# Fuad-HH/PumiUMTally

Measured on AMD Instinct MI355X. Metric: particle-steps/sec, higher is better.
Workload: dtype fp64; 1 GPU; model=track-length-tally-walk, mesh_tets=998250, global_batch=10000000, particles_per_gpu=10000000, parallelism=dp1-replicated-mesh, nscores=1, comm=torch-rccl, ngroups=1, device=gpu, lost_particles=0

## Files before the change

### csrc/core/engine.h

```cpp
#pragma once

#include "mesh.h"
#include "walk.h"

#include <cstdint>
#include <cstdlib>
#include <stdexcept>
#include <memory>
#include <string>
#include <vector>

namespace pumitally {

struct EngineStats {
  int64_t lost_particles = 0;
  int64_t moves = 0;
  int64_t relocated = 0;
  int64_t loose_localizations = 0;
  int64_t origins_elided = 0;
  int64_t origin_bytes_uploaded = 0;
  double origin_pass_seconds = 0.0;
  int64_t collisions_scored = 0;
  int64_t collision_misses = 0;
};

constexpr int kMaxLostRecords = 16;

class Engine {
public:
  virtual ~Engine() = default;

  virtual int64_t num_particles() const = 0;
  virtual const Mesh &mesh() const = 0;

  virtual void copy_initial_position(const double *positions, int64_t n) = 0;

  virtual void move(const double *origin, const double *dest,
                    const int8_t *flying, const double *weights, int64_t n,
                    const uint16_t *groups = nullptr,
                    const double *responses = nullptr) = 0;

  virtual void move_continue(const double *dest, const int8_t *flying,
                             const double *weights, int64_t n,
                             const uint16_t *groups = nullptr,
                             const double *responses = nullptr) {
    move(nullptr, dest, flying, weights, n, groups, responses);
  }

  virtual void move_device(const double *d_origin, const double *d_dest,
                           const int8_t *d_flying, const double *d_weights,
                           int64_t n, const uint16_t *d_groups = nullptr,
                           const double *d_responses = nullptr) {
    (void)d_origin; (void)d_dest; (void)d_flying; (void)d_weights; (void)n;
    (void)d_groups; (void)d_responses;
// ... 105 lines not shown
  virtual void set_particle_state(const double *pos, const int32_t *elem,
                                  const uint8_t *escaped, int64_t n) = 0;

  virtual void synchronize() {}

  struct DeviceMeshView {
    const Plane *planes = nullptr;
    const int32_t *nbr = nullptr;
    GridView grid{};
    void *stream = nullptr;
  };
  virtual bool device_mesh(DeviceMeshView *out) const {
    (void)out;
    return false;
  }

  int max_steps = 0;
  int ngroups = 1;
  int nscores = 1;

  bool reflective = false;

  bool linear = false;

  bool face_currents = false;

  bool collision_tallies = false;

  bool walk_fp32 = false;

  bool origin_elide = true;
  int origin_threads = 8;
  int64_t origin_chunk = 0;

protected:
  [[noreturn]] static void throw_not_linear() {
    throw std::runtime_error(
        "linear moment tallies are off: create the engine with linear=true");
  }
  [[noreturn]] static void throw_not_currents() {
    throw std::runtime_error(
        "face-current tallies are off: create the engine with currents=true");
  }
  [[noreturn]] static void throw_not_collisions() {
    throw std::runtime_error(
        "collision tallies are off: create the engine with collisions=true");
  }
};

inline bool default_walk_fp32() {
  const char *s = getenv("PUMITALLY_WALK");
  return s && std::string(s) == "fp32";
}

inline bool default_origin_elide() {
  const char *s = getenv("PUMITALLY_ORIGIN_ELIDE");
  return !s || atoi(s) != 0;
}

inline int default_origin_threads() {
  const char *s = getenv("PUMITALLY_ORIGIN_THREADS");
  const int k = s ? atoi(s) : 8;
  return k < 1 ? 1 : (k > 16 ? 16 : k);
}

inline int64_t default_origin_chunk() {
  const char *s = getenv("PUMITALLY_ORIGIN_CHUNK");
  const int64_t c = s ? (int64_t)atoll(s) : 0;
  return c < 0 ? 0 : c;
}

inline bool default_reflective() {
  const char *s = getenv("PUMITALLY_BC");
  return s && std::string(s) == "reflective";
}

inline double loc_tol_rel() {
  const char *s = getenv("PUMITALLY_LOC_TOL");
  return s ? atof(s) : 1e-10;
}

std::unique_ptr<Engine> make_cpu_engine(Mesh mesh, int64_t num_particles,
                                        int ngroups = 1, int nscores = 1,
                                        bool linear = false,
                                        bool currents = false,
                                        bool collisions = false);

std::unique_ptr<Engine> make_gpu_engine(Mesh mesh, int64_t num_particles,
                                        int device, int ngroups = 1,
                                        int nscores = 1, bool linear = false,
                                        bool currents = false,
                                        bool collisions = false);

inline void check_tally_options(bool linear, bool currents) {
  if (linear && currents)
    throw std::invalid_argument(
        "currents=true cannot be combined with linear=true (not implemented)");
}

std::vector<double> normalize_flux(const Mesh &m, const std::vector<double> &flux);
// ... 8 lines not shown
```

### csrc/core/origin_delta.cpp

```cpp
#include "origin_delta.h"

#include <algorithm>
#include <atomic>
#include <cstring>

#if defined(__SSE2__) && !defined(__HIP_DEVICE_COMPILE__)
#include <emmintrin.h>
#define PT_HAVE_STREAM_STORE 1
#else
#define PT_HAVE_STREAM_STORE 0
#endif

namespace pumitally {

int origin_delta_clamp_threads(int requested) {
  return std::max(1, std::min(requested, kOriginDeltaMaxThreads));
}

OriginDeltaPool::OriginDeltaPool(int nthreads)
    : nthreads_(origin_delta_clamp_threads(nthreads)) {
  for (int t = 1; t < nthreads_; ++t)
    threads_.emplace_back([this, t] { worker(t); });
}

// ... 73 lines not shown
  _mm_sfence();
#endif
}

template <bool NT>
int64_t delta_part(const double *origin, const double *dest, double *shadow,
                   int64_t lo, int64_t hi, int32_t *pidx, double *pxyz,
                   int64_t cap) {
  int64_t count = 0;
  for (int64_t i = lo; i < hi; ++i) {
    const double *o = origin + i * 3;
    double *s = shadow + i * 3;
    const uint64_t diff = (load_bits(o) ^ load_bits(s)) |
                          (load_bits(o + 1) ^ load_bits(s + 1)) |
                          (load_bits(o + 2) ^ load_bits(s + 2));
    if (diff) {
      if (count < cap) {
        pidx[count] = (int32_t)i;
        pxyz[count * 3] = o[0];
        pxyz[count * 3 + 1] = o[1];
        pxyz[count * 3 + 2] = o[2];
      }
      ++count;
    }
    const double *d = dest + i * 3;
    store_bits<NT>(s, load_bits(d));
    store_bits<NT>(s + 1, load_bits(d + 1));
    store_bits<NT>(s + 2, load_bits(d + 2));
  }
  if (NT) store_fence();
  return count;
}

template <bool NT>
void copy_part(const double *dest, double *shadow, int64_t lo, int64_t hi) {
  for (int64_t k = lo * 3; k < hi * 3; ++k)
    store_bits<NT>(shadow + k, load_bits(dest + k));
  if (NT) store_fence();
}

}

int64_t origin_delta_block(int64_t len, int nthreads) {
  const int64_t t = origin_delta_clamp_threads(nthreads);
  const int64_t b = (len + 4 * t - 1) / (4 * t);
  return std::max<int64_t>(1, std::min(b, kMaxBlock));
}

int64_t origin_delta_patch_capacity(int64_t len, int nthreads) {
  if (len <= 0) return 0;
  const int64_t block = origin_delta_block(len, nthreads);
  const int64_t full = len / block, tail = len % block;
  return full * seg_capacity(block) + (tail ? seg_capacity(tail) : 0);
}

OriginDeltaResult origin_delta_pass(OriginDeltaPool &pool,
                                    const double *origin, const double *dest,
                                    double *shadow, int64_t lo, int64_t hi,
                                    int32_t *patch_idx, double *patch_xyz,
                                    bool nontemporal) {
  OriginDeltaResult r;
  const int64_t len = hi - lo;
  if (len <= 0) return r;
  r.block = origin_delta_block(len, pool.nthreads());
  r.nsegs = (len + r.block - 1) / r.block;
  r.seg_off.resize(r.nsegs);
  r.seg_cap.resize(r.nsegs);
  r.seg_count.assign(r.nsegs, 0);
  for (int64_t b = 0; b < r.nsegs; ++b) {
    const int64_t blen = std::min(r.block, len - b * r.block);
    r.seg_off[b] = b * seg_capacity(r.block);
    r.seg_cap[b] = seg_capacity(blen);
  }
  std::atomic<int64_t> next{0};
  const std::function<void(int)> job = [&](int) {
    for (;;) {
      const int64_t b = next.fetch_add(1, std::memory_order_relaxed);
      if (b >= r.nsegs) return;
      const int64_t a = lo + b * r.block;
      const int64_t e = std::min(hi, a + r.block);
      int32_t *pi = patch_idx + r.seg_off[b];
      double *px = patch_xyz + r.seg_off[b] * 3;
      r.seg_count[b] =
          nontemporal
              ? delta_part<true>(origin, dest, shadow, a, e, pi, px,
                                 r.seg_cap[b])
              : delta_part<false>(origin, dest, shadow, a, e, pi, px,
                                  r.seg_cap[b]);
    }
  };
  pool.run(job);
  for (int64_t b = 0; b < r.nsegs; ++b) {
    r.changed += r.seg_count[b];
    if (r.seg_count[b] > r.seg_cap[b]) r.overflow = true;
  }
  return r;
}

void origin_delta_compact(const OriginDeltaResult &r, int32_t *patch_idx,
                          double *patch_xyz) {
  int64_t out = 0;
  for (int64_t b = 0; b < r.nsegs; ++b) {
    const int64_t cnt = r.seg_count[b];
    if (cnt && r.seg_off[b] != out) {
      std::memmove(patch_idx + out, patch_idx + r.seg_off[b],
                   cnt * sizeof(int32_t));
      std::memmove(patch_xyz + out * 3, patch_xyz + r.seg_off[b] * 3,
                   cnt * 3 * sizeof(double));
    }
    out += cnt;
  }
}

void origin_delta_seed(OriginDeltaPool &pool, const double *dest,
                       double *shadow, int64_t lo, int64_t hi,
                       bool nontemporal) {
  const int64_t len = hi - lo;
  if (len <= 0) return;
  const int64_t block = origin_delta_block(len, pool.nthreads());
  const int64_t nblocks = (len + block - 1) / block;
  std::atomic<int64_t> next{0};
  const std::function<void(int)> job = [&](int) {
    for (;;) {
      const int64_t b = next.fetch_add(1, std::memory_order_relaxed);
      if (b >= nblocks) return;
      const int64_t a = lo + b * block;
      const int64_t e = std::min(hi, a + block);
      if (nontemporal)
        copy_part<true>(dest, shadow, a, e);
      else
        copy_part<false>(dest, shadow, a, e);
    }
  };
  pool.run(job);
}

}
```

### csrc/core/origin_delta.h

```cpp
#pragma once

#include <condition_variable>
#include <cstdint>
#include <functional>
#include <mutex>
#include <thread>
#include <vector>

namespace pumitally {

constexpr int kOriginDeltaMaxThreads = 16;

int origin_delta_clamp_threads(int requested);

class OriginDeltaPool {
public:
  explicit OriginDeltaPool(int nthreads);
  ~OriginDeltaPool();
  OriginDeltaPool(const OriginDeltaPool &) = delete;
  OriginDeltaPool &operator=(const OriginDeltaPool &) = delete;

  int nthreads() const { return nthreads_; }
  void run(const std::function<void(int)> &f);

// ... 6 lines not shown
  std::condition_variable cv_start_, cv_done_;
  const std::function<void(int)> *job_ = nullptr;
  uint64_t generation_ = 0;
  int pending_ = 0;
  bool stop_ = false;
};

struct OriginDeltaResult {
  int64_t block = 0;
  int64_t nsegs = 0;
  std::vector<int64_t> seg_off, seg_cap;
  std::vector<int64_t> seg_count;
  int64_t changed = 0;
  bool overflow = false;
};

int64_t origin_delta_block(int64_t len, int nthreads);

int64_t origin_delta_patch_capacity(int64_t len, int nthreads);

OriginDeltaResult origin_delta_pass(OriginDeltaPool &pool,
                                    const double *origin, const double *dest,
                                    double *shadow, int64_t lo, int64_t hi,
                                    int32_t *patch_idx, double *patch_xyz,
                                    bool nontemporal = false);

void origin_delta_compact(const OriginDeltaResult &r, int32_t *patch_idx,
                          double *patch_xyz);

void origin_delta_seed(OriginDeltaPool &pool, const double *dest,
                       double *shadow, int64_t lo, int64_t hi,
                       bool nontemporal = false);

}
```

### csrc/hip/engine_gpu.hip

```cpp
#include "../core/engine.h"
#include "../core/origin_delta.h"
#include "../core/tally_sink.h"
#include "../core/walk.h"
#include "hip_util.h"

#include <hip/hip_runtime.h>
#include <hipcub/hipcub.hpp>

#include <algorithm>
#include <type_traits>
#include <array>
#include <chrono>
#include <cstdio>
#include <cstdlib>
#include <cstring>
#include <memory>
#include <stdexcept>
#include <string>
#include <vector>

namespace pumitally {

namespace {

// ... 691 lines not shown
      d_flying_[p].allocate(n_);
      d_weights_[p].allocate(n_);
      if (ngroups > 1) d_groups_[p].allocate(n_);
    }

    sort_every_ = sort_every();
    if (sort_every_ > 0) {
      d_keys_.allocate(n_);
      d_keys2_.allocate(n_);
      d_vals_.allocate(n_);
      d_order_.allocate(n_);
      d_pos2_.allocate(n_ * 3);
      d_elem2_.allocate(n_);
      d_esc2_.allocate(n_);
      d_s2c2_.allocate(n_);
      size_t bytes = 0;
      PT_HIP_CHECK(hipcub::DeviceRadixSort::SortPairs(
          nullptr, bytes, d_keys_.get(), d_keys2_.get(), d_vals_.get(),
          d_order_.get(), (int)n_, 0, 64, s_comp_));
      sorttmp_bytes_ = bytes;
      d_sorttmp_.allocate(bytes ? bytes : 1);
      const Vec3 ext = mesh_.bbox_hi - mesh_.bbox_lo;
      sort_scale_ = Vec3{ext.x > 0 ? 2097151.0 / ext.x : 0.0,
                         ext.y > 0 ? 2097151.0 / ext.y : 0.0,
                         ext.z > 0 ? 2097151.0 / ext.z : 0.0};
    }

    loc_tol_ = loc_tol_rel() * norm(mesh_.bbox_hi - mesh_.bbox_lo);
    walk_fp32 = default_walk_fp32();
    reflective = default_reflective();
    origin_elide = default_origin_elide();
    origin_threads = default_origin_threads();
    origin_chunk = default_origin_chunk();
    const Vec3 c0 = mesh_.nelems > 0 ? mesh_.centroid(0) : Vec3{0, 0, 0};
    k_init_particles<<<grid_blocks(n_), kBlock, 0, s_comp_>>>(
        d_pos_, d_elem_, d_escaped_, d_s2c_, n_, c0.x, c0.y, c0.z);
    PT_HIP_CHECK(hipGetLastError());
    PT_HIP_CHECK(hipStreamSynchronize(s_comp_));
  }

  ~GpuEngine() override {
    (void)hipSetDevice(device_);
    (void)hipDeviceSynchronize();
  }

  int64_t num_particles() const override { return n_; }
  const Mesh &mesh() const override { return mesh_; }

  void copy_initial_position(const double *p, int64_t n) override {
    check_n(n);
    PT_HIP_CHECK(hipSetDevice(device_));
    sync();
    stage(p, n * 3 * sizeof(double), d_origin_[0], s_copy_);
    PT_HIP_CHECK(hipStreamSynchronize(s_copy_));
    k_iota<<<grid_blocks(n_), kBlock, 0, s_comp_>>>(d_s2c_, n_);
    k_locate<<<grid_blocks(n_), kBlock, 0, s_comp_>>>(
        d_planes_, grid_view_, d_origin_[0], d_pos_, d_elem_, d_escaped_,
        d_loose_, n_, loc_tol_);
    PT_HIP_CHECK(hipGetLastError());
    if (sort_every_ > 0) spatial_sort();
    moves_since_sort_ = 0;
    PT_HIP_CHECK(hipStreamSynchronize(s_comp_));
  }

  void move(const double *origin, const double *dest, const int8_t *flying,
            const double *weights, int64_t n,
            const uint16_t *groups = nullptr,
            const double *responses = nullptr) override {
    check_n(n);
    PT_HIP_CHECK(hipSetDevice(device_));
    const int steps = max_steps > 0 ? max_steps : default_max_steps(mesh_);
    const int p = (int)(parity_++ & 1);
    PT_HIP_CHECK(hipStreamWaitEvent(s_copy_, kernels_done_[p], 0));
    if (responses && !d_resp_[p]) d_resp_[p].allocate(n_ * nscores);
    const bool probe = origin && origin_elide && n > 0 && elide_skip_ == 0;
    if (probe && shadow_valid_) {
      stage_elided(p, origin, dest, flying, weights, groups, responses, n);
    } else {
      if (origin) {
        stage(origin, n * 3 * sizeof(double), d_origin_[p], s_copy_);
        stats_.origin_bytes_uploaded += n * 3 * (int64_t)sizeof(double);
      }
      stage_inputs(p, dest, flying, weights, groups, responses, n);
      shadow_valid_ = false;
      if (probe) {
        ensure_elide_host(n);
        const auto t0 = std::chrono::steady_clock::now();
        origin_delta_seed(*delta_pool_, dest, shadow_.get(), 0, n,
                          false);
        stats_.origin_pass_seconds += seconds_since(t0);
        shadow_valid_ = true;
      } else if (origin && origin_elide && elide_skip_ > 0) {
        --elide_skip_;
      }
    }
    PT_HIP_CHECK(hipEventRecord(copy_ev_[p], s_copy_));
    PT_HIP_CHECK(hipStreamWaitEvent(s_comp_, copy_ev_[p], 0));
    launch_move_chunks(origin ? d_origin_[p] : nullptr, d_dest_[p],
                       d_flying_[p], d_weights_[p],
                       groups ? d_groups_[p] : nullptr,
                       responses ? d_resp_[p] : nullptr, n, steps);
    PT_HIP_CHECK(hipEventRecord(kernels_done_[p], s_comp_));
    maybe_resort();
    PT_HIP_CHECK(hipStreamSynchronize(s_copy_));
    stats_.moves++;
  }

  void move_device(const double *d_origin, const double *d_dest,
                   const int8_t *d_flying, const double *d_weights, int64_t n,
                   const uint16_t *d_groups = nullptr,
                   const double *d_responses = nullptr) override {
    check_n(n);
    PT_HIP_CHECK(hipSetDevice(device_));
    const int steps = max_steps > 0 ? max_steps : default_max_steps(mesh_);
    launch_move_chunks(d_origin, d_dest, d_flying, d_weights, d_groups,
                       d_responses, n, steps);
    maybe_resort();
    stats_.moves++;
  }

  void score_collisions(const int8_t *active, const double *weights,
                        int64_t n, const uint16_t *groups = nullptr,
                        const double *responses = nullptr) override {
// ... 390 lines not shown
    PT_HIP_CHECK(hipStreamSynchronize(s_comp_));
    PT_HIP_CHECK(hipMemcpy(d_pos_, pos, n * 3 * sizeof(double), hipMemcpyHostToDevice));
    PT_HIP_CHECK(hipMemcpy(d_elem_, elem, n * sizeof(int32_t), hipMemcpyHostToDevice));
    PT_HIP_CHECK(hipMemcpy(d_escaped_, escaped, n, hipMemcpyHostToDevice));
    moves_since_sort_ = sort_every_;
  }

  void synchronize() override { sync(); }

  bool device_mesh(DeviceMeshView *out) const override {
    out->planes = d_planes_;
    out->nbr = d_nbr_;
    out->grid = grid_view_;
    out->stream = (void *)s_comp_;
    return true;
  }

private:
  void check_n(int64_t n) const {
    if (n != n_) throw std::runtime_error("particle count mismatch");
  }

  void sync() const {
    PT_HIP_CHECK(hipStreamSynchronize(s_copy_));
    PT_HIP_CHECK(hipStreamSynchronize(s_comp_));
  }

  void stage(const void *src, size_t bytes, void *dst, hipStream_t s) {
    PT_HIP_CHECK(hipMemcpyAsync(dst, src, bytes, hipMemcpyHostToDevice, s));
  }

  void stage_inputs(int p, const double *dest, const int8_t *flying,
                    const double *weights, const uint16_t *groups,
                    const double *responses, int64_t n) {
    stage(dest, n * 3 * sizeof(double), d_dest_[p], s_copy_);
    stage(flying, n * sizeof(int8_t), d_flying_[p], s_copy_);
    stage(weights, n * sizeof(double), d_weights_[p], s_copy_);
    if (groups && d_groups_[p])
      stage(groups, n * sizeof(uint16_t), d_groups_[p], s_copy_);
    if (responses)
      stage(responses, n * nscores * sizeof(double), d_resp_[p], s_copy_);
  }

  static constexpr int kElideBackoffFirst = 16;
  static constexpr int kElideBackoffMax = 256;

  static double seconds_since(std::chrono::steady_clock::time_point t0) {
    return std::chrono::duration<double>(std::chrono::steady_clock::now() -
                                         t0)
        .count();
  }

  int64_t elide_chunk(int64_t n) const {
    if (origin_chunk > 0) return std::max<int64_t>(origin_chunk, 64);
    return std::max<int64_t>((int64_t)262144, (n + 1) / 2);
  }

  void ensure_elide_host(int64_t n) {
    const int want = origin_delta_clamp_threads(origin_threads);
    if (!delta_pool_ || delta_pool_->nthreads() != want)
      delta_pool_ = std::make_unique<OriginDeltaPool>(want);
    if (!shadow_) shadow_.reset(new double[n * 3]);
  }

  void ensure_patch(int64_t need) {
    if (need <= patch_cap_) return;
    PT_HIP_CHECK(hipStreamSynchronize(s_copy_));
    patch_cap_ = 0;
    h_patch_idx_.reset();
    h_patch_xyz_.reset();
    d_patch_idx_.reset();
    d_patch_xyz_.reset();
    h_patch_idx_.allocate(need);
    h_patch_xyz_.allocate(need * 3);
    d_patch_idx_.allocate(need);
    d_patch_xyz_.allocate(need * 3);
    patch_cap_ = need;
  }

  void stage_elided(int p, const double *origin, const double *dest,
                    const int8_t *flying, const double *weights,
                    const uint16_t *groups, const double *responses,
                    int64_t n) {
    ensure_elide_host(n);
    const int nthreads = delta_pool_->nthreads();
    const int64_t chunk = elide_chunk(n);
    int64_t need = 0;
    for (int64_t lo = 0; lo < n; lo += chunk)
      need += origin_delta_patch_capacity(std::min(chunk, n - lo), nthreads);
    ensure_patch(need);
    shadow_valid_ = false;
    k_copy_doubles<<<grid_blocks(n * 3 / 2), kBlock, 0, s_copy_>>>(
        d_dest_[p ^ 1], d_origin_[p], n * 3);
    PT_HIP_CHECK(hipGetLastError());
    stage_inputs(p, dest, flying, weights, groups, responses, n);
    int64_t region = 0, uploaded = 0;
    for (int64_t lo = 0; lo < n; lo += chunk) {
      const int64_t hi = std::min(n, lo + chunk);
      const int64_t len = hi - lo;
      const int64_t cap = origin_delta_patch_capacity(len, nthreads);
      if (region + cap > patch_cap_)
        throw std::runtime_error("origin elision: patch region overflow");
      int32_t *hidx = h_patch_idx_ + region;
      double *hxyz = h_patch_xyz_ + region * 3;
      const auto t0 = std::chrono::steady_clock::now();
      const OriginDeltaResult r = origin_delta_pass(
          *delta_pool_, origin, dest, shadow_.get(), lo, hi, hidx, hxyz,
          false);
      stats_.origin_pass_seconds += seconds_since(t0);
      if (r.overflow || r.changed * 2 > len) {
        stage(origin + lo * 3, len * 3 * sizeof(double),
              d_origin_[p] + lo * 3, s_copy_);
        uploaded += len;
      } else if (r.changed > 0) {
        origin_delta_compact(r, hidx, hxyz);
        stage(hidx, r.changed * sizeof(int32_t), d_patch_idx_ + region,
              s_copy_);
        stage(hxyz, r.changed * 3 * sizeof(double),
              d_patch_xyz_ + region * 3, s_copy_);
        k_scatter_origins<<<grid_blocks(r.changed), kBlock, 0, s_copy_>>>(
            d_patch_idx_ + region, d_patch_xyz_ + region * 3, d_origin_[p],
            r.changed);
        PT_HIP_CHECK(hipGetLastError());
        uploaded += r.changed;
      }
      region += cap;
    }
    stats_.origins_elided += n - uploaded;
    stats_.origin_bytes_uploaded += uploaded * 3 * (int64_t)sizeof(double);
    shadow_valid_ = true;
    if (uploaded * 2 > n) {
      elide_skip_ = elide_backoff_;
      elide_backoff_ = std::min(elide_backoff_ * 2, kElideBackoffMax);
    } else {
      elide_backoff_ = kElideBackoffFirst;
    }
  }

  void launch_walk_raw(int64_t n, const double *pos, const double *dest,
                       const int32_t *elem, const double *weights,
                       double *out_pos, int32_t *out_elem, int8_t *out_status,
// ... 84 lines not shown
    }
  }

  template <class T>
  std::pair<std::vector<int32_t>, std::vector<T>> fetch(const T *dev,
                                                        int comps) const {
    sync();
    std::vector<int32_t> s2c(n_);
    std::vector<T> v(n_ * comps);
    PT_HIP_CHECK(hipMemcpy(s2c.data(), d_s2c_, n_ * sizeof(int32_t),
                           hipMemcpyDeviceToHost));
    PT_HIP_CHECK(hipMemcpy(v.data(), dev, n_ * comps * sizeof(T),
                           hipMemcpyDeviceToHost));
    return {std::move(s2c), std::move(v)};
  }

  Mesh mesh_;
  int64_t n_;
  int64_t fsz_ = 0;
  int device_ = 0;
  double loc_tol_ = 1e-12;
  int slices_ = 1;
  int sort_every_ = 0;
  int64_t moves_since_sort_ = 0;
  uint64_t parity_ = 0;
  Vec3 sort_scale_{0, 0, 0};

  std::unique_ptr<double[]> shadow_;
  bool shadow_valid_ = false;
  std::unique_ptr<OriginDeltaPool> delta_pool_;
  int64_t patch_cap_ = 0;
  int elide_skip_ = 0;
  int elide_backoff_ = kElideBackoffFirst;

  Stream s_copy_, s_comp_;
  std::array<Event, 2> copy_ev_;
  std::array<Event, 2> kernels_done_;
  Stream s_score_;
  Event score_copied_, score_done_;
  bool score_queued_ = false;

  PinnedBuffer<int32_t> h_patch_idx_;
  PinnedBuffer<double> h_patch_xyz_;
  DeviceBuffer<int32_t> d_patch_idx_;
  DeviceBuffer<double> d_patch_xyz_;

  DeviceBuffer<Plane> d_planes_;
  DeviceBuffer<Plane32> d_planes32_;
  DeviceBuffer<int32_t> d_nbr_, d_cell_start_, d_cell_tets_;
  GridView grid_view_{};

  DeviceBuffer<double> d_pos_;
  DeviceBuffer<int32_t> d_elem_;
  DeviceBuffer<uint8_t> d_escaped_;
  DeviceBuffer<int32_t> d_s2c_;
  DeviceBuffer<double> d_flux_;
  DeviceBuffer<unsigned long long> d_lost_, d_loose_;
  DeviceBuffer<double> d_lostrec_;
  DeviceBuffer<double> d_origin_[2], d_dest_[2], d_weights_[2], d_resp_[2];
  DeviceBuffer<int8_t> d_flying_[2];
  DeviceBuffer<uint16_t> d_groups_[2];
  DeviceBuffer<double> d_bsum_, d_bsq_;
  DeviceBuffer<double> d_inv_h_, d_moments_, d_msum_;
  DeviceBuffer<double> d_cur_, d_csum_, d_csq_;
  bool cur_keyed_ = false;
  DeviceBuffer<double> d_coll_, d_collsum_, d_collsq_;
  DeviceBuffer<unsigned long long> d_coll_counts_;
  bool coll_agg_ = true;
  DeviceBuffer<int8_t> sc_active_;
  DeviceBuffer<double> sc_weights_, sc_resp_;
  DeviceBuffer<uint16_t> sc_groups_;
  ScorePointsScratch sp_;
  DeviceBuffer<uint32_t> d_face_bc_;
  DeviceBuffer<int32_t> d_pidx_, d_pelem_;
// ... 35 lines not shown
```

### csrc/pybind/module.cpp

```cpp
#include <pybind11/numpy.h>
#include <pybind11/pybind11.h>
#include <pybind11/stl.h>

#include "../api/PumiTally.h"
#include "../comm/comm.h"
#include "../core/engine.h"
#include "../core/partition_engine.h"

#include <hip/hip_runtime.h>

#include <cstdint>
#include <cstring>
#include <memory>
#include <thread>
#include <vector>

namespace py = pybind11;
using namespace pumitally;

namespace {

bool have_gpu() {
  int n = 0;
  if (hipGetDeviceCount(&n) != hipSuccess) {
// ... 673 lines not shown
           py::arg("ngroups") = 1, py::arg("nscores") = 1,
           py::arg("linear") = false, py::arg("currents") = false,
           py::arg("collisions") = false)
      .def_property_readonly(
          "collision_tallies",
          [](const PyEngine &e) { return e.eng->collision_tallies; })
      .def_property_readonly("linear",
                             [](const PyEngine &e) { return e.eng->linear; })
      .def_property_readonly(
          "face_currents",
          [](const PyEngine &e) { return e.eng->face_currents; })
      .def_property_readonly(
          "reflective", [](const PyEngine &e) { return e.eng->reflective; })
      .def_property_readonly("ngroups",
                             [](const PyEngine &e) { return e.eng->ngroups; })
      .def_property_readonly("nscores",
                             [](const PyEngine &e) { return e.eng->nscores; })
      .def_property_readonly("num_particles",
                             [](const PyEngine &e) { return e.eng->num_particles(); })
      .def_property_readonly("is_gpu", [](const PyEngine &e) { return e.gpu; })
      .def_property(
          "max_steps", [](const PyEngine &e) { return e.eng->max_steps; },
          [](PyEngine &e, int v) { e.eng->max_steps = v; })
      .def_property(
          "origin_elide", [](const PyEngine &e) { return e.eng->origin_elide; },
          [](PyEngine &e, bool v) { e.eng->origin_elide = v; })
      .def_property(
          "origin_threads",
          [](const PyEngine &e) { return e.eng->origin_threads; },
          [](PyEngine &e, int v) { e.eng->origin_threads = v; })
      .def_property(
          "origin_chunk", [](const PyEngine &e) { return e.eng->origin_chunk; },
          [](PyEngine &e, int64_t v) { e.eng->origin_chunk = v; })
      .def("copy_initial_position",
           [](PyEngine &e, py::array_t<double, py::array::c_style | py::array::forcecast> p) {
             if ((int64_t)p.size() != e.eng->num_particles() * 3)
               throw std::runtime_error("positions must have size 3*num_particles");
             e.eng->copy_initial_position(p.data(), e.eng->num_particles());
           })
      .def("move",
           [](PyEngine &e, py::array_t<double, py::array::c_style> origin,
              py::array_t<double, py::array::c_style> dest,
              py::array_t<int8_t, py::array::c_style> flying,
              py::array_t<double, py::array::c_style> weights,
              py::object groups, py::object responses) {
             const int64_t n = e.eng->num_particles();
             if ((int64_t)origin.size() != n * 3 || (int64_t)dest.size() != n * 3 ||
                 (int64_t)flying.size() != n || (int64_t)weights.size() != n)
               throw std::runtime_error("move: array size mismatch");
             const uint16_t *gp = nullptr;
             py::array_t<uint16_t, py::array::c_style | py::array::forcecast> garr;
             if (!groups.is_none()) {
               garr = groups.cast<py::array_t<uint16_t, py::array::c_style | py::array::forcecast>>();
               if ((int64_t)garr.size() != n)
                 throw std::runtime_error("move: groups size mismatch");
               gp = garr.data();
             }
             const double *rp = nullptr;
             py::array_t<double, py::array::c_style | py::array::forcecast> rarr;
             if (!responses.is_none()) {
               rarr = responses.cast<py::array_t<double, py::array::c_style | py::array::forcecast>>();
               if ((int64_t)rarr.size() != n * e.eng->nscores)
                 throw std::runtime_error("move: responses size must be n*nscores");
               rp = rarr.data();
             }
             py::gil_scoped_release nogil;
// ... 248 lines not shown
           py::arg("groups_ptr") = 0, py::arg("responses_ptr") = 0)
      .def("collisions", [](const PyEngine &e) { return vec_to_np(e.eng->collisions()); })
      .def("collision_sum", [](const PyEngine &e) { return vec_to_np(e.eng->collision_sum()); })
      .def("collision_sum_sq", [](const PyEngine &e) { return vec_to_np(e.eng->collision_sum_sq()); })
      .def("set_collisions",
           [](PyEngine &e, py::array_t<double, py::array::c_style | py::array::forcecast> c) {
             e.eng->set_collisions(c.data(), (int64_t)c.size());
           })
      .def("set_particle_state",
           [](PyEngine &e, py::array_t<double, py::array::c_style | py::array::forcecast> pos,
              py::array_t<int32_t, py::array::c_style | py::array::forcecast> elem,
              py::array_t<uint8_t, py::array::c_style | py::array::forcecast> escaped) {
             const int64_t n = e.eng->num_particles();
             if ((int64_t)pos.size() != n * 3 || (int64_t)elem.size() != n ||
                 (int64_t)escaped.size() != n)
               throw std::runtime_error("set_particle_state: size mismatch");
             e.eng->set_particle_state(pos.data(), elem.data(), escaped.data(), n);
           })
      .def("end_batch", [](PyEngine &e) { py::gil_scoped_release ng; e.eng->end_batch(); })
      .def("batch_sum", [](const PyEngine &e) { return vec_to_np(e.eng->batch_sum()); })
      .def("batch_sum_sq", [](const PyEngine &e) { return vec_to_np(e.eng->batch_sum_sq()); })
      .def_property_readonly("num_batches",
                             [](const PyEngine &e) { return e.eng->num_batches(); })
      .def("stats", [](const PyEngine &e) {
        const EngineStats &s = e.eng->stats();
        py::dict d;
        d["lost_particles"] = s.lost_particles;
        d["moves"] = s.moves;
        d["relocated"] = s.relocated;
        d["loose_localizations"] = s.loose_localizations;
        d["origins_elided"] = s.origins_elided;
        d["origin_bytes_uploaded"] = s.origin_bytes_uploaded;
        d["origin_pass_seconds"] = s.origin_pass_seconds;
        d["collisions_scored"] = s.collisions_scored;
        d["collision_misses"] = s.collision_misses;
        return d;
      })
      .def("lost_records", [](const PyEngine &e) {
        auto v = e.eng->lost_records();
        auto arr = vec_to_np(std::move(v));
        return arr.reshape({(py::ssize_t)(arr.size() / 4), (py::ssize_t)4});
      });

  py::class_<PumiTally>(m, "PumiTally")
      .def(py::init([](const std::string &mesh, int32_t n) {
        int argc = 0;
        char **argv = nullptr;
        return new PumiTally(mesh, n, argc, argv);
      }))
      .def("copy_initial_position",
           [](PumiTally &t, py::array_t<double, py::array::c_style | py::array::forcecast> p) {
             t.CopyInitialPosition((double *)p.data(), (int32_t)p.size());
           })
      .def("move_to_next_location",
           [](PumiTally &t, py::array_t<double, py::array::c_style> origin,
              py::array_t<double, py::array::c_style> dest,
              py::array_t<int8_t, py::array::c_style> flying,
              py::array_t<double, py::array::c_style> weights) {
             t.MoveToNextLocation((double *)origin.data(), (double *)dest.data(),
                                  (int8_t *)flying.mutable_data(),
                                  (double *)weights.data(), (int32_t)origin.size());
           })
      .def("write_tally_results", &PumiTally::WriteTallyResults)
      .def("tally_times", [](const PumiTally &t) {
        py::dict d;
        d["initialization_time"] = t.InitializationTime();
// ... 6 lines not shown
```

### pumiumtally_amd/__init__.py

```python
from __future__ import annotations

import os as _os

if _os.environ.get("PUMITALLY_NO_TORCH", "0") != "1":
    try:
        import torch as _torch
    except ImportError:
        pass


def _load_core():
    try:
        from . import _core
        return _core
    except ImportError as e:
        if _os.environ.get("PUMITALLY_AUTOBUILD", "1") == "1":
            from ._build import build
            build()
            from . import _core
            return _core
        raise ImportError(
            "pumiumtally_amd._core is not built. Run "
            "`python -m pumiumtally_amd._build` first."
        ) from e
# ... 74 lines not shown
        return self._eng.is_gpu

    @property
    def max_steps(self) -> int:
        return self._eng.max_steps

    @max_steps.setter
    def max_steps(self, v: int) -> None:
        self._eng.max_steps = v

    @property
    def origin_elide(self) -> bool:
        return self._eng.origin_elide

    @origin_elide.setter
    def origin_elide(self, v: bool) -> None:
        self._eng.origin_elide = bool(v)

    @property
    def origin_threads(self) -> int:
        return self._eng.origin_threads

    @origin_threads.setter
    def origin_threads(self, v: int) -> None:
        self._eng.origin_threads = int(v)

    @property
    def origin_chunk(self) -> int:
        return self._eng.origin_chunk

    @origin_chunk.setter
    def origin_chunk(self, v: int) -> None:
        self._eng.origin_chunk = int(v)

    def copy_initial_position(self, positions):
        self._eng.copy_initial_position(positions)

    def move(self, origin, dest, flying, weights, groups=None,
             responses=None):
        self._eng.move(origin, dest, flying, weights, groups, responses)

    def move_continue(self, dest, flying, weights, groups=None,
                      responses=None):
        self._eng.move_continue(dest, flying, weights, groups, responses)

    def move_from_device(self, dest, flying, weights, origin=None,
                         sync_torch=True, groups=None, responses=None):
        def ptr(t, dtype, numel):
            return _device_ptr(t, dtype, numel, "move_from_device")

        n = self.num_particles
        if sync_torch:
            _sync_torch()
        self._eng.move_device(
            ptr(origin, "<f8", n * 3), ptr(dest, "<f8", n * 3),
            ptr(flying, "|i1", n), ptr(weights, "<f8", n),
            ptr(groups, "<u2", n), ptr(responses, "<f8", n * self.nscores))

    def walk_raw(self, pos, dest, elem, weights, groups=None,
                 responses=None, in_t=None, in_prev=None, resume=False):
        return self._eng.walk_raw(pos, dest, elem, weights, groups,
                                  responses, in_t, in_prev, resume)

    def synchronize(self):
        self._eng.synchronize()

# ... 396 lines not shown
```

Measured before the change: 1.401 billion particle-steps/s.

## Echo uploaded dest back to pinned host and elide unchanged flying/weight uploads

```diff
diff --git a/csrc/core/engine.h b/csrc/core/engine.h
--- a/csrc/core/engine.h
+++ b/csrc/core/engine.h
@@ -20,6 +20,11 @@
   int64_t origins_elided = 0;
   int64_t origin_bytes_uploaded = 0;
   double origin_pass_seconds = 0.0;
+  double origin_echo_wait_seconds = 0.0;
+  int64_t origin_echo_fallbacks = 0;
+  int64_t weight_bytes_uploaded = 0;
+  int64_t flying_bytes_uploaded = 0;
+  double input_pass_seconds = 0.0;
   int64_t collisions_scored = 0;
   int64_t collision_misses = 0;
 };
@@ -191,6 +196,9 @@
   bool origin_elide = true;
   int origin_threads = 8;
   int64_t origin_chunk = 0;
+  bool origin_echo = true;
+  bool input_elide = true;
+  int64_t input_block = 0;
 
 protected:
   [[noreturn]] static void throw_not_linear() {
@@ -225,6 +233,22 @@
 
 inline int64_t default_origin_chunk() {
   const char *s = getenv("PUMITALLY_ORIGIN_CHUNK");
+  const int64_t c = s ? (int64_t)atoll(s) : 0;
+  return c < 0 ? 0 : c;
+}
+
+inline bool default_origin_echo() {
+  const char *s = getenv("PUMITALLY_ORIGIN_ECHO");
+  return !s || atoi(s) != 0;
+}
+
+inline bool default_input_elide() {
+  const char *s = getenv("PUMITALLY_INPUT_ELIDE");
+  return !s || atoi(s) != 0;
+}
+
+inline int64_t default_input_block() {
+  const char *s = getenv("PUMITALLY_INPUT_BLOCK");
   const int64_t c = s ? (int64_t)atoll(s) : 0;
   return c < 0 ? 0 : c;
 }
diff --git a/csrc/core/origin_delta.cpp b/csrc/core/origin_delta.cpp
--- a/csrc/core/origin_delta.cpp
+++ b/csrc/core/origin_delta.cpp
@@ -129,6 +129,28 @@
   return count;
 }
 
+int64_t compare_part(const double *origin, const double *prev, int64_t lo,
+                     int64_t hi, int32_t *pidx, double *pxyz, int64_t cap) {
+  int64_t count = 0;
+  for (int64_t i = lo; i < hi; ++i) {
+    const double *o = origin + i * 3;
+    const double *s = prev + i * 3;
+    const uint64_t diff = (load_bits(o) ^ load_bits(s)) |
+                          (load_bits(o + 1) ^ load_bits(s + 1)) |
+                          (load_bits(o + 2) ^ load_bits(s + 2));
+    if (diff) {
+      if (count < cap) {
+        pidx[count] = (int32_t)i;
+        pxyz[count * 3] = o[0];
+        pxyz[count * 3 + 1] = o[1];
+        pxyz[count * 3 + 2] = o[2];
+      }
+      ++count;
+    }
+  }
+  return count;
+}
+
 template <bool NT>
 void copy_part(const double *dest, double *shadow, int64_t lo, int64_t hi) {
   for (int64_t k = lo * 3; k < hi * 3; ++k)
@@ -151,11 +173,12 @@
   return full * seg_capacity(block) + (tail ? seg_capacity(tail) : 0);
 }
 
-OriginDeltaResult origin_delta_pass(OriginDeltaPool &pool,
-                                    const double *origin, const double *dest,
-                                    double *shadow, int64_t lo, int64_t hi,
-                                    int32_t *patch_idx, double *patch_xyz,
-                                    bool nontemporal) {
+namespace {
+
+template <class Part>
+OriginDeltaResult run_pass(OriginDeltaPool &pool, int64_t lo, int64_t hi,
+                           int32_t *patch_idx, double *patch_xyz,
+                           const Part &part) {
   OriginDeltaResult r;
   const int64_t len = hi - lo;
   if (len <= 0) return r;
@@ -176,14 +199,8 @@
       if (b >= r.nsegs) return;
       const int64_t a = lo + b * r.block;
       const int64_t e = std::min(hi, a + r.block);
-      int32_t *pi = patch_idx + r.seg_off[b];
-      double *px = patch_xyz + r.seg_off[b] * 3;
-      r.seg_count[b] =
-          nontemporal
-              ? delta_part<true>(origin, dest, shadow, a, e, pi, px,
-                                 r.seg_cap[b])
-              : delta_part<false>(origin, dest, shadow, a, e, pi, px,
-                                  r.seg_cap[b]);
+      r.seg_count[b] = part(a, e, patch_idx + r.seg_off[b],
+                            patch_xyz + r.seg_off[b] * 3, r.seg_cap[b]);
     }
   };
   pool.run(job);
@@ -192,6 +209,35 @@
     if (r.seg_count[b] > r.seg_cap[b]) r.overflow = true;
   }
   return r;
+}
+
+}
+
+OriginDeltaResult origin_delta_pass(OriginDeltaPool &pool,
+                                    const double *origin, const double *dest,
+                                    double *shadow, int64_t lo, int64_t hi,
+                                    int32_t *patch_idx, double *patch_xyz,
+                                    bool nontemporal) {
+  return run_pass(pool, lo, hi, patch_idx, patch_xyz,
+                  [&](int64_t a, int64_t e, int32_t *pi, double *px,
+                      int64_t cap) {
+                    return nontemporal ? delta_part<true>(origin, dest, shadow,
+                                                          a, e, pi, px, cap)
+                                       : delta_part<false>(origin, dest, shadow,
+                                                           a, e, pi, px, cap);
+                  });
+}
+
+OriginDeltaResult origin_delta_compare(OriginDeltaPool &pool,
+                                       const double *origin,
+                                       const double *prev, int64_t lo,
+                                       int64_t hi, int32_t *patch_idx,
+                                       double *patch_xyz) {
+  return run_pass(pool, lo, hi, patch_idx, patch_xyz,
+                  [&](int64_t a, int64_t e, int32_t *pi, double *px,
+                      int64_t cap) {
+                    return compare_part(origin, prev, a, e, pi, px, cap);
+                  });
 }
 
 void origin_delta_compact(const OriginDeltaResult &r, int32_t *patch_idx,
@@ -232,4 +278,48 @@
   pool.run(job);
 }
 
-}
+int64_t input_delta_block(int64_t n, int64_t requested) {
+  if (requested > 0) return requested;
+  (void)n;
+  return 4096;
+}
+
+InputDeltaResult input_delta_blocks(OriginDeltaPool &pool, const void *cur,
+                                    void *shadow, int64_t n, int64_t elem_size,
+                                    int64_t block) {
+  InputDeltaResult r;
+  if (n <= 0) return r;
+  r.block = std::max<int64_t>(1, block);
+  r.nblocks = (n + r.block - 1) / r.block;
+  r.differs.assign(r.nblocks, 0);
+  const int64_t per_claim = std::max<int64_t>(1, 65536 / r.block);
+  const char *c = static_cast<const char *>(cur);
+  char *s = static_cast<char *>(shadow);
+  std::atomic<int64_t> next{0};
+  const std::function<void(int)> job = [&](int) {
+    for (;;) {
+      const int64_t b0 = next.fetch_add(per_claim, std::memory_order_relaxed);
+      if (b0 >= r.nblocks) return;
+      const int64_t b1 = std::min(r.nblocks, b0 + per_claim);
+      for (int64_t b = b0; b < b1; ++b) {
+        const int64_t a = b * r.block;
+        const size_t bytes =
+            (size_t)((std::min(n, a + r.block) - a) * elem_size);
+        if (std::memcmp(c + a * elem_size, s + a * elem_size, bytes) != 0) {
+          std::memcpy(s + a * elem_size, c + a * elem_size, bytes);
+          r.differs[b] = 1;
+        }
+      }
+    }
+  };
+  pool.run(job);
+  for (int64_t b = 0; b < r.nblocks; ++b) {
+    if (!r.differs[b]) continue;
+    ++r.changed_blocks;
+    r.changed_elems += std::min(n, (b + 1) * r.block) - b * r.block;
+    if (b == 0 || !r.differs[b - 1]) ++r.runs;
+  }
+  return r;
+}
+
+}
diff --git a/csrc/core/origin_delta.h b/csrc/core/origin_delta.h
--- a/csrc/core/origin_delta.h
+++ b/csrc/core/origin_delta.h
@@ -62,4 +62,25 @@
                        double *shadow, int64_t lo, int64_t hi,
                        bool nontemporal = false);
 
+OriginDeltaResult origin_delta_compare(OriginDeltaPool &pool,
+                                       const double *origin,
+                                       const double *prev, int64_t lo,
+                                       int64_t hi, int32_t *patch_idx,
+                                       double *patch_xyz);
+
+struct InputDeltaResult {
+  int64_t block = 0;
+  int64_t nblocks = 0;
+  std::vector<uint8_t> differs;
+  int64_t changed_blocks = 0;
+  int64_t changed_elems = 0;
+  int64_t runs = 0;
+};
+
+int64_t input_delta_block(int64_t n, int64_t requested);
+
+InputDeltaResult input_delta_blocks(OriginDeltaPool &pool, const void *cur,
+                                    void *shadow, int64_t n, int64_t elem_size,
+                                    int64_t block);
+
 }
diff --git a/csrc/hip/engine_gpu.hip b/csrc/hip/engine_gpu.hip
--- a/csrc/hip/engine_gpu.hip
+++ b/csrc/hip/engine_gpu.hip
@@ -747,6 +747,9 @@
     origin_elide = default_origin_elide();
     origin_threads = default_origin_threads();
     origin_chunk = default_origin_chunk();
+    origin_echo = default_origin_echo();
+    input_elide = default_input_elide();
+    input_block = default_input_block();
     const Vec3 c0 = mesh_.nelems > 0 ? mesh_.centroid(0) : Vec3{0, 0, 0};
     k_init_particles<<<grid_blocks(n_), kBlock, 0, s_comp_>>>(
         d_pos_, d_elem_, d_escaped_, d_s2c_, n_, c0.x, c0.y, c0.z);
@@ -787,23 +790,32 @@
     const int steps = max_steps > 0 ? max_steps : default_max_steps(mesh_);
     const int p = (int)(parity_++ & 1);
     PT_HIP_CHECK(hipStreamWaitEvent(s_copy_, kernels_done_[p], 0));
+    if (echo_pieces_[p] > 0)
+      PT_HIP_CHECK(hipStreamWaitEvent(
+          s_copy_, echo_done_[p][echo_pieces_[p] - 1], 0));
     if (responses && !d_resp_[p]) d_resp_[p].allocate(n_ * nscores);
     const bool probe = origin && origin_elide && n > 0 && elide_skip_ == 0;
-    if (probe && shadow_valid_) {
-      stage_elided(p, origin, dest, flying, weights, groups, responses, n);
+    const bool echo = probe && origin_echo && ensure_echo();
+    if (probe && shadow_valid_ && prev_in_echo_ == echo) {
+      stage_elided(p, origin, dest, flying, weights, groups, responses, n,
+                   echo);
     } else {
       if (origin) {
         stage(origin, n * 3 * sizeof(double), d_origin_[p], s_copy_);
         stats_.origin_bytes_uploaded += n * 3 * (int64_t)sizeof(double);
       }
-      stage_inputs(p, dest, flying, weights, groups, responses, n);
+      stage_inputs(p, dest, flying, weights, groups, responses, n, echo);
       shadow_valid_ = false;
-      if (probe) {
+      if (echo) {
+        prev_in_echo_ = true;
+        shadow_valid_ = true;
+      } else if (probe) {
         ensure_elide_host(n);
         const auto t0 = std::chrono::steady_clock::now();
         origin_delta_seed(*delta_pool_, dest, shadow_.get(), 0, n,
                           false);
         stats_.origin_pass_seconds += seconds_since(t0);
+        prev_in_echo_ = false;
         shadow_valid_ = true;
       } else if (origin && origin_elide && elide_skip_ > 0) {
         --elide_skip_;
@@ -1260,16 +1272,137 @@
 
   void stage_inputs(int p, const double *dest, const int8_t *flying,
                     const double *weights, const uint16_t *groups,
-                    const double *responses, int64_t n) {
-    stage(dest, n * 3 * sizeof(double), d_dest_[p], s_copy_);
-    stage(flying, n * sizeof(int8_t), d_flying_[p], s_copy_);
-    stage(weights, n * sizeof(double), d_weights_[p], s_copy_);
+                    const double *responses, int64_t n, bool echo = false) {
+    if (echo)
+      stage_dest_echoed(p, dest, n);
+    else
+      stage(dest, n * 3 * sizeof(double), d_dest_[p], s_copy_);
+    stage_flying_weights(p, flying, weights, n);
     if (groups && d_groups_[p])
       stage(groups, n * sizeof(uint16_t), d_groups_[p], s_copy_);
     if (responses)
       stage(responses, n * nscores * sizeof(double), d_resp_[p], s_copy_);
   }
 
+  static constexpr int kInputMaxCopies = 64;
+
+  void ensure_input_shadows(int64_t n) {
+    ensure_pool();
+    if (!w_shadow_) {
+      w_shadow_.reset(new double[n]());
+      f_shadow_.reset(new int8_t[n]());
+    }
+  }
+
+  bool stage_input_array(const InputDeltaResult &r, const void *src,
+                         void *dst, const void *dst_prev, int64_t n,
+                         int64_t elem, int64_t *bytes_uploaded) {
+    if (!inputs_valid_ || r.changed_elems * 2 > n ||
+        r.runs > kInputMaxCopies) {
+      stage(src, n * elem, dst, s_copy_);
+      *bytes_uploaded += n * elem;
+      return true;
+    }
+    if (elem == (int64_t)sizeof(double)) {
+      k_copy_doubles<<<grid_blocks((n + 1) / 2), kBlock, 0, s_copy_>>>(
+          (const double *)dst_prev, (double *)dst, n);
+      PT_HIP_CHECK(hipGetLastError());
+    } else {
+      PT_HIP_CHECK(hipMemcpyAsync(dst, dst_prev, n * elem,
+                                  hipMemcpyDeviceToDevice, s_copy_));
+    }
+    for (int64_t b = 0; b < r.nblocks;) {
+      if (!r.differs[b]) {
+        ++b;
+        continue;
+      }
+      int64_t e = b + 1;
+      while (e < r.nblocks && r.differs[e]) ++e;
+      const int64_t lo = b * r.block, hi = std::min(n, e * r.block);
+      stage((const char *)src + lo * elem, (hi - lo) * elem,
+            (char *)dst + lo * elem, s_copy_);
+      *bytes_uploaded += (hi - lo) * elem;
+      b = e;
+    }
+    return false;
+  }
+
+  void stage_flying_weights(int p, const int8_t *flying, const double *weights,
+                            int64_t n) {
+    if (!input_elide || n <= 0 || input_skip_ > 0) {
+      stage(flying, n * sizeof(int8_t), d_flying_[p], s_copy_);
+      stage(weights, n * sizeof(double), d_weights_[p], s_copy_);
+      stats_.flying_bytes_uploaded += n * (int64_t)sizeof(int8_t);
+      stats_.weight_bytes_uploaded += n * (int64_t)sizeof(double);
+      inputs_valid_ = false;
+      if (input_elide && input_skip_ > 0) --input_skip_;
+      return;
+    }
+    ensure_input_shadows(n);
+    const int64_t block = input_delta_block(n, input_block);
+    const auto t0 = std::chrono::steady_clock::now();
+    const InputDeltaResult rf = input_delta_blocks(
+        *delta_pool_, flying, f_shadow_.get(), n, sizeof(int8_t), block);
+    const InputDeltaResult rw = input_delta_blocks(
+        *delta_pool_, weights, w_shadow_.get(), n, sizeof(double), block);
+    stats_.input_pass_seconds += seconds_since(t0);
+    const bool f_whole =
+        stage_input_array(rf, flying, d_flying_[p], d_flying_[p ^ 1], n,
+                          sizeof(int8_t), &stats_.flying_bytes_uploaded);
+    const bool w_whole =
+        stage_input_array(rw, weights, d_weights_[p], d_weights_[p ^ 1], n,
+                          sizeof(double), &stats_.weight_bytes_uploaded);
+    if (inputs_valid_ && (f_whole || w_whole)) {
+      input_skip_ = input_backoff_;
+      input_backoff_ = std::min(input_backoff_ * 2, kElideBackoffMax);
+    } else if (inputs_valid_) {
+      input_backoff_ = kElideBackoffFirst;
+    }
+    inputs_valid_ = true;
+  }
+
+  static constexpr int kEchoPieces = 4;
+
+  bool ensure_echo() {
+    if (echo_ready_) return true;
+    if (echo_failed_) return false;
+    try {
+      h_echo_[0].allocate(n_ * 3);
+      h_echo_[1].allocate(n_ * 3);
+    } catch (const std::runtime_error &) {
+      (void)hipGetLastError();
+      h_echo_[0].reset();
+      h_echo_[1].reset();
+      echo_failed_ = true;
+      ++stats_.origin_echo_fallbacks;
+      return false;
+    }
+    s_echo_.create();
+    for (auto &evs : dest_up_)
+      for (auto &ev : evs) ev.create();
+    for (auto &evs : echo_done_)
+      for (auto &ev : evs) ev.create();
+    echo_ready_ = true;
+    return true;
+  }
+
+  void stage_dest_echoed(int p, const double *dest, int64_t n) {
+    const int64_t piece = (n + kEchoPieces - 1) / kEchoPieces;
+    int pieces = 0;
+    for (int64_t lo = 0; lo < n; lo += piece, ++pieces) {
+      const int64_t len = std::min(piece, n - lo);
+      const size_t bytes = (size_t)len * 3 * sizeof(double);
+      stage(dest + lo * 3, bytes, d_dest_[p] + lo * 3, s_copy_);
+      PT_HIP_CHECK(hipEventRecord(dest_up_[p][pieces], s_copy_));
+      PT_HIP_CHECK(hipStreamWaitEvent(s_echo_, dest_up_[p][pieces], 0));
+      PT_HIP_CHECK(hipMemcpyAsync(h_echo_[p] + lo * 3, d_dest_[p] + lo * 3,
+                                  bytes, hipMemcpyDeviceToHost, s_echo_));
+      PT_HIP_CHECK(hipEventRecord(echo_done_[p][pieces], s_echo_));
+    }
+    echo_piece_len_[p] = piece;
+    echo_pieces_[p] = pieces;
+  }
+
   static constexpr int kElideBackoffFirst = 16;
   static constexpr int kElideBackoffMax = 256;
 
@@ -1284,10 +1417,14 @@
     return std::max<int64_t>((int64_t)262144, (n + 1) / 2);
   }
 
-  void ensure_elide_host(int64_t n) {
+  void ensure_pool() {
     const int want = origin_delta_clamp_threads(origin_threads);
     if (!delta_pool_ || delta_pool_->nthreads() != want)
       delta_pool_ = std::make_unique<OriginDeltaPool>(want);
+  }
+
+  void ensure_elide_host(int64_t n) {
+    ensure_pool();
     if (!shadow_) shadow_.reset(new double[n * 3]);
   }
 
@@ -1309,8 +1446,13 @@
   void stage_elided(int p, const double *origin, const double *dest,
                     const int8_t *flying, const double *weights,
                     const uint16_t *groups, const double *responses,
-                    int64_t n) {
-    ensure_elide_host(n);
+                    int64_t n, bool echo) {
+    if (echo)
+      ensure_pool();
+    else
+      ensure_elide_host(n);
+    const int q = p ^ 1;
+    int echo_synced = 0;
     const int nthreads = delta_pool_->nthreads();
     const int64_t chunk = elide_chunk(n);
     int64_t need = 0;
@@ -1321,7 +1463,7 @@
     k_copy_doubles<<<grid_blocks(n * 3 / 2), kBlock, 0, s_copy_>>>(
         d_dest_[p ^ 1], d_origin_[p], n * 3);
     PT_HIP_CHECK(hipGetLastError());
-    stage_inputs(p, dest, flying, weights, groups, responses, n);
+    stage_inputs(p, dest, flying, weights, groups, responses, n, echo);
     int64_t region = 0, uploaded = 0;
     for (int64_t lo = 0; lo < n; lo += chunk) {
       const int64_t hi = std::min(n, lo + chunk);
@@ -1331,10 +1473,20 @@
         throw std::runtime_error("origin elision: patch region overflow");
       int32_t *hidx = h_patch_idx_ + region;
       double *hxyz = h_patch_xyz_ + region * 3;
+      if (echo) {
+        const int upto = (int)((hi - 1) / echo_piece_len_[q]);
+        const auto tw = std::chrono::steady_clock::now();
+        for (; echo_synced <= upto; ++echo_synced)
+          PT_HIP_CHECK(hipEventSynchronize(echo_done_[q][echo_synced]));
+        stats_.origin_echo_wait_seconds += seconds_since(tw);
+      }
       const auto t0 = std::chrono::steady_clock::now();
-      const OriginDeltaResult r = origin_delta_pass(
-          *delta_pool_, origin, dest, shadow_.get(), lo, hi, hidx, hxyz,
-          false);
+      const OriginDeltaResult r =
+          echo ? origin_delta_compare(*delta_pool_, origin, h_echo_[q].get(),
+                                      lo, hi, hidx, hxyz)
+               : origin_delta_pass(*delta_pool_, origin, dest, shadow_.get(),
+                                   lo, hi, hidx, hxyz,
+                                   false);
       stats_.origin_pass_seconds += seconds_since(t0);
       if (r.overflow || r.changed * 2 > len) {
         stage(origin + lo * 3, len * 3 * sizeof(double),
@@ -1485,6 +1637,15 @@
   int64_t patch_cap_ = 0;
   int elide_skip_ = 0;
   int elide_backoff_ = kElideBackoffFirst;
+  bool prev_in_echo_ = false;
+  bool echo_ready_ = false, echo_failed_ = false;
+  int64_t echo_piece_len_[2] = {1, 1};
+  int echo_pieces_[2] = {0, 0};
+  std::unique_ptr<double[]> w_shadow_;
+  std::unique_ptr<int8_t[]> f_shadow_;
+  bool inputs_valid_ = false;
+  int input_skip_ = 0;
+  int input_backoff_ = kElideBackoffFirst;
 
   Stream s_copy_, s_comp_;
   std::array<Event, 2> copy_ev_;
@@ -1492,7 +1653,10 @@
   Stream s_score_;
   Event score_copied_, score_done_;
   bool score_queued_ = false;
-
+  std::array<std::array<Event, kEchoPieces>, 2> dest_up_, echo_done_;
+  Stream s_echo_;
+
+  PinnedBuffer<double> h_echo_[2];
   PinnedBuffer<int32_t> h_patch_idx_;
   PinnedBuffer<double> h_patch_xyz_;
   DeviceBuffer<int32_t> d_patch_idx_;
diff --git a/csrc/pybind/module.cpp b/csrc/pybind/module.cpp
--- a/csrc/pybind/module.cpp
+++ b/csrc/pybind/module.cpp
@@ -729,6 +729,15 @@
       .def_property(
           "origin_chunk", [](const PyEngine &e) { return e.eng->origin_chunk; },
           [](PyEngine &e, int64_t v) { e.eng->origin_chunk = v; })
+      .def_property(
+          "origin_echo", [](const PyEngine &e) { return e.eng->origin_echo; },
+          [](PyEngine &e, bool v) { e.eng->origin_echo = v; })
+      .def_property(
+          "input_elide", [](const PyEngine &e) { return e.eng->input_elide; },
+          [](PyEngine &e, bool v) { e.eng->input_elide = v; })
+      .def_property(
+          "input_block", [](const PyEngine &e) { return e.eng->input_block; },
+          [](PyEngine &e, int64_t v) { e.eng->input_block = v < 0 ? 0 : v; })
       .def("copy_initial_position",
            [](PyEngine &e, py::array_t<double, py::array::c_style | py::array::forcecast> p) {
              if ((int64_t)p.size() != e.eng->num_particles() * 3)
@@ -1043,6 +1052,11 @@
         d["origins_elided"] = s.origins_elided;
         d["origin_bytes_uploaded"] = s.origin_bytes_uploaded;
         d["origin_pass_seconds"] = s.origin_pass_seconds;
+        d["origin_echo_wait_seconds"] = s.origin_echo_wait_seconds;
+        d["origin_echo_fallbacks"] = s.origin_echo_fallbacks;
+        d["weight_bytes_uploaded"] = s.weight_bytes_uploaded;
+        d["flying_bytes_uploaded"] = s.flying_bytes_uploaded;
+        d["input_pass_seconds"] = s.input_pass_seconds;
         d["collisions_scored"] = s.collisions_scored;
         d["collision_misses"] = s.collision_misses;
         return d;
diff --git a/pumiumtally_amd/__init__.py b/pumiumtally_amd/__init__.py
--- a/pumiumtally_amd/__init__.py
+++ b/pumiumtally_amd/__init__.py
@@ -130,6 +130,30 @@
     @origin_chunk.setter
     def origin_chunk(self, v: int) -> None:
         self._eng.origin_chunk = int(v)
+
+    @property
+    def origin_echo(self) -> bool:
+        return self._eng.origin_echo
+
+    @origin_echo.setter
+    def origin_echo(self, v: bool) -> None:
+        self._eng.origin_echo = bool(v)
+
+    @property
+    def input_elide(self) -> bool:
+        return self._eng.input_elide
+
+    @input_elide.setter
+    def input_elide(self, v: bool) -> None:
+        self._eng.input_elide = bool(v)
+
+    @property
+    def input_block(self) -> int:
+        return self._eng.input_block
+
+    @input_block.setter
+    def input_block(self, v: int) -> None:
+        self._eng.input_block = int(v)
 
     def copy_initial_position(self, positions):
         self._eng.copy_initial_position(positions)
```

Measured after the change: 1.615 billion particle-steps/s, median of 4. 15.3% higher.
